# Wendison/FCL-taco2

Hardware: AMD Instinct MI355X
Metric: mel-frames/sec (FCL-taco2-S forward, batch=32, 80-mel) (higher is better)
Workload: dtype f32 via bf16x3-split MFMA operands, fp32 accumulate (max-abs 8e-6 on mel vs the reference; FCL_PRECISION=0 = exact fp32 MFMA)

## Files before the change

fcl-taco2_amd/csrc/decoder_step.hip:

```cpp
#include "fcl_common.h"
#include "lstm_epilogue.h"

namespace fcl {


template <int NT>
__device__ __forceinline__ void rowtile_mma(const float* A_l, int lda_l, const float* const (&wrow)[NT], int K, int r16, int kq,
                                            f32x4 (&out)[NT], int rot = 0) {
    f32x4 acc0[NT], acc1[NT];
#pragma unroll
    for (int t = 0; t < NT; ++t) acc0[t] = acc1[t] = (f32x4){0.f, 0.f, 0.f, 0.f};
    const float* ap = A_l + r16 * lda_l + kq * 4;
    const float* wp[NT];
#pragma unroll
    for (int t = 0; t < NT; ++t) wp[t] = wrow[t] + kq * 4;
    const int nfull = K >> 6;
    f32x4 bn[NT][4];
    int cc = nfull > 0 ? rot % nfull : 0;
    if (nfull > 0) {
#pragma unroll
        for (int t = 0; t < NT; ++t)
#pragma unroll
            for (int i = 0; i < 4; ++i) bn[t][i] = *reinterpret_cast<const f32x4*>(wp[t] + (cc << 6) + i * 16);
    }
// ... 253 lines not shown
            for (int e = 0; e < 4; ++e) split1(v[j][e], h[e], l[e]);
            *reinterpret_cast<uint2*>(Ah + r * ldk + c) = make_uint2(h[0] | ((unsigned)h[1] << 16), h[2] | ((unsigned)h[3] << 16));
            *reinterpret_cast<uint2*>(Al + r * ldk + c) = make_uint2(l[0] | ((unsigned)l[1] << 16), l[2] | ((unsigned)l[3] << 16));
        }
    }
    __device__ __forceinline__ void store(float* dst, int ld_l) const {
#pragma unroll
        for (int j = 0; j < 4; ++j) {
            const int i = threadIdx.x + j * 256, r = i >> 6, c = (i & 63) * 4;
            *reinterpret_cast<f32x4*>(dst + r * ld_l + c) = v[j];
        }
    }
};

__global__ __launch_bounds__(512) void feat_prenet_x3_kernel(const FeatPrenetArgs a) {
    const int M_feat = a.M_feat, M_pre = a.M_pre;
    const int Ms_feat = (a.live && a.t_prev >= 0) ? min(a.M_feat, a.live[a.t_prev]) : a.M_feat, Ms_pre = a.live ? min(a.M_pre, a.live[a.t_cur]) : a.M_pre;
    if (a.live && a.w0 && blockIdx.x == 0 && threadIdx.x == 0 && a.live[a.t_cur] > a.M_pre) atomicOr(a.status, (unsigned int)FCL_STATUS_ROWS_CAP);
    if ((int)blockIdx.x * (16) >= (a.h1 ? Ms_feat : Ms_pre)) return;
    extern __shared__ __attribute__((aligned(16))) float smem[];
    const int ldU = a.U + 8, ldO = a.O + 8, ldP = a.P + 8;
    u16* A1h = reinterpret_cast<u16*>(smem);
    u16* A1l = A1h + 16 * ldU;
    u16* A2h = A1l + 16 * ldU;
    u16* A2l = A2h + 16 * ldO;
    u16* A3h = A2l + 16 * ldO;
    u16* A3l = A3h + 16 * ldP;
    const int m0 = blockIdx.x * 16;
    const int lane = threadIdx.x & 63, wave = threadIdx.x >> 6, nwaves = blockDim.x >> 6;
    const int r16 = lane & 15, kq = lane >> 4;
    const int col = lane & 15, rq = lane >> 4;
    const unsigned int sbump = a.seed_dev ? *a.seed_dev * 0x9E3779B9u : 0u;
    const unsigned int seed0 = hash_u32(a.seed0 + sbump), seed1 = hash_u32(a.seed1 + sbump);

    const bool has_pre = a.w0 && m0 < M_pre;
    const int ptile = wave, ptile2 = wave + nwaves;
    const int nsU = (a.U + 31) >> 5, nsO = (a.O + 31) >> 5, nsP = (a.P + 31) >> 5, ptmax = ((a.P + 15) >> 4) - 1;
    const size_t lane8 = (size_t)lane * 8;
    auto frag = [&](const u16* base, int tile, int ns) { return base + (size_t)tile * ns * 512 + lane8; };
    float pb0[2] = {0.f, 0.f}, pb1[2] = {0.f, 0.f};
    if (has_pre) {
#pragma unroll
        for (int tt = 0; tt < 2; ++tt) {
            const int nc = min((tt ? ptile2 : ptile) * 16 + col, a.P - 1);
            pb0[tt] = a.b0[nc];
            pb1[tt] = a.b1[nc];
        }
    }
    if (a.h1) {
        f32x4 accv[1];
        load_rowtile_split(A1h, A1l, ldU, a.h1, a.U, a.U, m0, M_feat);
        __syncthreads();
        for (int tile = wave; tile * 16 < a.O; tile += nwaves) {
            const u16* const wh[1] = {frag(a.wf_hi, tile, nsU)};
            const u16* const wl[1] = {frag(a.wf_lo, tile, nsU)};
            const int nc = tile * 16 + col, ncc = min(nc, a.O - 1);
            float f0v[4];
            int fo[4];
#pragma unroll
            for (int r = 0; r < 4; ++r) {
                const int mc = min(m0 + rq * 4 + r, M_feat - 1);
                f0v[r] = a.F0[(size_t)mc * a.O + ncc];
                fo[r] = a.frame_off[mc];
            }
            rowtile_mma_x3<1>(A1h, A1l, ldU, wh, wl, a.U, r16, kq, accv);
#pragma unroll
            for (int r = 0; r < 4; ++r) {
                const int row = rq * 4 + r, m = m0 + row;
                float v = 0.f;
                if (m < Ms_feat && nc < a.O) {
                    v = accv[0][r] + f0v[r];
                    a.before[(size_t)(fo[r] + a.t_prev) * a.O + nc] = v;
                    if (a.before_p) store_p32(a.before_p, (a.O + 31) >> 5, fo[r] + a.t_prev, nc, v);
                }
                if (nc < a.O) split1((a.out_act && m < Ms_feat) ? act_apply(v, a.out_act) : v, A2h[row * ldO + nc], A2l[row * ldO + nc]);
            }
        }
        if (a.before_p && (a.O & 31)) {
            const int padc = 32 - (a.O & 31);
            for (int i = threadIdx.x; i < 16 * padc; i += blockDim.x) {
                const int m = m0 + i / padc;
                if (m < Ms_feat) store_p32(a.before_p, (a.O + 31) >> 5, a.frame_off[m] + a.t_prev, a.O + i % padc, 0.f);
            }
        }
    } else {
        for (int i = threadIdx.x; i < 16 * ldO; i += blockDim.x) { A2h[i] = 0; A2l[i] = 0; }
    }
    if (!has_pre) return;
    lds_barrier();
    if (a.teacher_in) {
        load_rowtile_split(A2h, A2l, ldO, a.teacher_in, a.teacher_ld, a.O, m0, M_pre);
        __syncthreads();
    }
    for (int tile = wave; tile * 16 < a.P; tile += 2 * nwaves) {
        const int tile2 = tile + nwaves;
        const u16* const wh[2] = {frag(a.w0_hi, tile, nsO), frag(a.w0_hi, min(tile2, ptmax), nsO)};
        const u16* const wl[2] = {frag(a.w0_lo, tile, nsO), frag(a.w0_lo, min(tile2, ptmax), nsO)};
        f32x4 accv[2];
        rowtile_mma_x3<2>(A2h, A2l, ldO, wh, wl, a.O, r16, kq, accv);
#pragma unroll
        for (int tt = 0; tt < 2; ++tt) {
            const int nc = (tt ? tile2 : tile) * 16 + col;
            if (nc < a.P) {
                const float bn = tile == ptile ? pb0[tt] : a.b0[nc];
#pragma unroll
                for (int r = 0; r < 4; ++r) {
                    const int row = rq * 4 + r, m = m0 + row;
                    float v = fmaxf(accv[tt][r] + bn, 0.f);
                    if (m < M_pre) v = drop_apply(v, a.drop_mode, a.keep0, a.P, m, nc, a.P, a.keep_scale, a.drop_p, seed0);
                    split1(v, A3h[row * ldP + nc], A3l[row * ldP + nc]);
                }
            }
        }
    }
    lds_barrier();
    for (int tile = wave; tile * 16 < a.P; tile += 2 * nwaves) {
        const int tile2 = tile + nwaves;
        const u16* const wh[2] = {frag(a.w1_hi, tile, nsP), frag(a.w1_hi, min(tile2, ptmax), nsP)};
        const u16* const wl[2] = {frag(a.w1_lo, tile, nsP), frag(a.w1_lo, min(tile2, ptmax), nsP)};
        f32x4 accv[2];
        rowtile_mma_x3<2>(A3h, A3l, ldP, wh, wl, a.P, r16, kq, accv);
#pragma unroll
        for (int tt = 0; tt < 2; ++tt) {
            const int nc = (tt ? tile2 : tile) * 16 + col;
            if (nc < a.P) {
                const float bn = tile == ptile ? pb1[tt] : a.b1[nc];
#pragma unroll
                for (int r = 0; r < 4; ++r) {
                    const int m = m0 + rq * 4 + r;
                    if (m >= Ms_pre) continue;
                    float v = fmaxf(accv[tt][r] + bn, 0.f);
                    v = drop_apply(v, a.drop_mode, a.keep1, a.P, m, nc, a.P, a.keep_scale, a.drop_p, seed1);
                    if (a.pre_out) a.pre_out[(size_t)m * a.P + nc] = v;
                    if (a.pre_out_p) store_p32(a.pre_out_p, (a.P + 31) >> 5, m, nc, v);
                    if (a.tap_prenet) a.tap_prenet[(size_t)(a.frame_off[m] + a.t_cur) * a.P + nc] = v;
                }
            }
        }
    }
}

__device__ __forceinline__ void p32_store4(unsigned short* __restrict__ p, int ld, long long m, int n, uint2 hi, uint2 lo) {
    unsigned short* line = p + ((size_t)m * ld + (n >> 5)) * 64 + (n & 31);
    *reinterpret_cast<uint2*>(line) = hi;
    *reinterpret_cast<uint2*>(line + 32) = lo;
}

struct OpsX3 {
    static constexpr bool kPlanes = true, kUnitsInLane = false;
    static constexpr int PAD = 16, LDS_BYTES = 2 * sizeof(u16);
    struct W {
        const u16 *hi, *lo;
        __device__ __forceinline__ W at(size_t o, size_t o2 = 0) const { return {hi + o + o2, lo + o + o2}; }
    };
    struct Tile {
        u16 *h, *l;
        __device__ __forceinline__ Tile at(int o) const { return {h + o, l + o}; }
        static __device__ __forceinline__ Tile carve(u16*& p, int n) {
            u16* b = p;
            p += 2 * n;
            return {b, b + n};
        }
        template <int N>
        static __device__ __forceinline__ Tile fixed() {
            __shared__ __attribute__((aligned(16))) u16 A_h[N];
            __shared__ __attribute__((aligned(16))) u16 A_lo[N];
            return {A_h, A_lo};
        }
    };
    template <int NT, int NS>
    struct Frag {
        s16x8 hi[NT][NS], lo[NT][NS];
        template <int S0 = 0, int S1 = NS>
        __device__ __forceinline__ void load(const W (&w)[NT]) {
#pragma unroll
            for (int t = 0; t < NT; ++t)
#pragma unroll
                for (int st = S0; st < S1; ++st) {
                    hi[t][st] = *reinterpret_cast<const s16x8*>(w[t].hi + st * 512);
                    lo[t][st] = *reinterpret_cast<const s16x8*>(w[t].lo + st * 512);
                }
        }
        template <bool W_IS_A>
        __device__ __forceinline__ void chain(Tile A, int ldk, int r16, int kq, f32x4 (&out)[NT]) const {
            auto mfma = [](s16x8 w, s16x8 a, f32x4 c) {
                return W_IS_A ? __builtin_amdgcn_mfma_f32_16x16x32_bf16(w, a, c, 0, 0, 0) : __builtin_amdgcn_mfma_f32_16x16x32_bf16(a, w, c, 0, 0, 0);
            };
            f32x4 acc[NT];
#pragma unroll
            for (int t = 0; t < NT; ++t) acc[t] = (f32x4){0.f, 0.f, 0.f, 0.f};
            const u16* ah = A.h + r16 * ldk + kq * 8;
            const u16* al = A.l + r16 * ldk + kq * 8;
#pragma unroll
            for (int st = 0; st < NS; ++st) {
                const s16x8 a_hi = *reinterpret_cast<const s16x8*>(ah + st * 32);
                const s16x8 a_lo = *reinterpret_cast<const s16x8*>(al + st * 32);
#pragma unroll
                for (int t = 0; t < NT; ++t) acc[t] = mfma(hi[t][st], a_lo, acc[t]);
#pragma unroll
                for (int t = 0; t < NT; ++t) acc[t] = mfma(lo[t][st], a_hi, acc[t]);
#pragma unroll
                for (int t = 0; t < NT; ++t) acc[t] = mfma(hi[t][st], a_hi, acc[t]);
            }
#pragma unroll
            for (int t = 0; t < NT; ++t) out[t] = acc[t];
        }
        __device__ __forceinline__ void mma_t(Tile A, int ldk, int r16, int kq, f32x4 (&out)[NT]) const { chain<true>(A, ldk, r16, kq, out); }
        __device__ __forceinline__ void mma_small(Tile A, int ldk, int r16, int kq, f32x4 (&out)[NT]) const { chain<false>(A, ldk, r16, kq, out); }
    };
    static __device__ __forceinline__ u16* dynamic_lds() {
        extern __shared__ __attribute__((aligned(16))) u16 x3_lds[];
        return x3_lds;
    }
    static __device__ __forceinline__ W wf(const FeatPrenetArgs& a) { return {a.wf_hi, a.wf_lo}; }
    static __device__ __forceinline__ W w0(const FeatPrenetArgs& a) { return {a.w0_hi, a.w0_lo}; }
    static __device__ __forceinline__ W w1(const FeatPrenetArgs& a) { return {a.w1_hi, a.w1_lo}; }
    static __device__ __forceinline__ W w(const GemmTerm& t) { return {t.Whi, t.Wlo}; }
    static __device__ __forceinline__ void store4(Tile t, int row, int ld, int col, const f32x4 v) {
        uint2 h, l;
        split4(v, h, l);
        *reinterpret_cast<uint2*>(t.h + row * ld + col) = h;
        *reinterpret_cast<uint2*>(t.l + row * ld + col) = l;
    }
    static __device__ __forceinline__ void store_rows(const RowTile256& r, Tile t, int ld) { r.split_store(t.h, t.l, ld); }
    static __device__ __forceinline__ void zero(Tile t, int n) {
        for (int i = threadIdx.x; i < n / 8; i += 512) {
            reinterpret_cast<uint4*>(t.h)[i] = make_uint4(0, 0, 0, 0);
            reinterpret_cast<uint4*>(t.l)[i] = make_uint4(0, 0, 0, 0);
        }
    }
};

struct OpsF32 {
    static constexpr bool kPlanes = false, kUnitsInLane = true;
    static constexpr int PAD = 8, LDS_BYTES = sizeof(float);
    struct W {
        const float* f;
        __device__ __forceinline__ W at(size_t o, size_t o2 = 0) const { return {f + o + o2}; }
    };
    struct Tile {
        float* p;
        __device__ __forceinline__ Tile at(int o) const { return {p + o}; }
        static __device__ __forceinline__ Tile carve(float*& p, int n) {
            float* b = p;
            p += n;
            return {b};
        }
        template <int N>
        static __device__ __forceinline__ Tile fixed() {
            __shared__ __attribute__((aligned(16))) float A_f[N];
            return {A_f};
        }
    };
    template <int NT, int NS>
    struct Frag {
        f32x4 w0[NT][NS], w1[NT][NS];
        template <int S0 = 0, int S1 = NS>
        __device__ __forceinline__ void load(const W (&w)[NT]) {
#pragma unroll
            for (int t = 0; t < NT; ++t)
#pragma unroll
                for (int st = S0; st < S1; ++st) {
                    w0[t][st] = *reinterpret_cast<const f32x4*>(w[t].f + st * 512);
                    w1[t][st] = *reinterpret_cast<const f32x4*>(w[t].f + st * 512 + 4);
                }
        }
        __device__ __forceinline__ void mma_t(Tile A, int ldk, int r16, int kq, f32x4 (&out)[NT]) const {
            f32x4 acc[NT];
#pragma unroll
            for (int t = 0; t < NT; ++t) acc[t] = (f32x4){0.f, 0.f, 0.f, 0.f};
            const float* a = A.p + r16 * ldk + kq * 4;
#pragma unroll
            for (int st = 0; st < NS; ++st) {
                const f32x4 a0 = *reinterpret_cast<const f32x4*>(a + st * 32), a1 = *reinterpret_cast<const f32x4*>(a + st * 32 + 16);
#pragma unroll
                for (int e = 0; e < 4; ++e)
#pragma unroll
                    for (int t = 0; t < NT; ++t) acc[t] = __builtin_amdgcn_mfma_f32_16x16x4f32(w0[t][st][e], a0[e], acc[t], 0, 0, 0);
#pragma unroll
                for (int e = 0; e < 4; ++e)
#pragma unroll
                    for (int t = 0; t < NT; ++t) acc[t] = __builtin_amdgcn_mfma_f32_16x16x4f32(w1[t][st][e], a1[e], acc[t], 0, 0, 0);
            }
#pragma unroll
            for (int t = 0; t < NT; ++t) out[t] = acc[t];
        }
        __device__ __forceinline__ void mma_small(Tile A, int ldk, int r16, int kq, f32x4 (&out)[NT]) const { mma_t(A, ldk, r16, kq, out); }
    };
    static __device__ __forceinline__ float* dynamic_lds() {
        extern __shared__ __attribute__((aligned(16))) float f32_lds[];
        return f32_lds;
    }
    static __device__ __forceinline__ W wf(const FeatPrenetArgs& a) { return {a.wf_ff}; }
    static __device__ __forceinline__ W w0(const FeatPrenetArgs& a) { return {a.w0_ff}; }
    static __device__ __forceinline__ W w1(const FeatPrenetArgs& a) { return {a.w1_ff}; }
    static __device__ __forceinline__ W w(const GemmTerm& t) { return {t.Wff}; }
    static __device__ __forceinline__ void store4(Tile t, int row, int ld, int col, const f32x4 v) { *reinterpret_cast<f32x4*>(t.p + row * ld + col) = v; }
    static __device__ __forceinline__ void store_rows(const RowTile256& r, Tile t, int ld) { r.store(t.p, ld); }
    static __device__ __forceinline__ void zero(Tile t, int n) {
        for (int i = threadIdx.x; i < n / 4; i += 512) reinterpret_cast<f32x4*>(t.p)[i] = (f32x4){0.f, 0.f, 0.f, 0.f};
    }
};

template <class Ops, int DROP, int RT>
__global__ __launch_bounds__(512) void feat_prenet_split_kernel(const FeatPrenetArgs a) {
    typedef typename Ops::Tile Tile;
    constexpr int SU = 8, SO = 3, SP = 8, U = 256, OP = 96, P = 256;
    const int M_feat = a.M_feat, M_pre = a.M_pre;
    int Ms_feat, Ms_pre;
    if (!feat_prenet_rows(a, 16 * RT, Ms_feat, Ms_pre)) return;
    constexpr int ldU = U + Ops::PAD, ldO = OP + Ops::PAD, ldP = P + Ops::PAD, ROWS = 16 * RT;
    static_assert(ldU == ldP, "the layer-1 operand tile re-uses the h1 tile's LDS");
    auto* lds = Ops::dynamic_lds();
    const Tile A1 = Tile::carve(lds, ROWS * ldU);
    const Tile A2 = Tile::carve(lds, ROWS * ldO);
    const Tile A3 = A1;
    const int O = a.O;
    const int m0 = blockIdx.x * ROWS;
    const int lane = threadIdx.x & 63, wave = __builtin_amdgcn_readfirstlane(threadIdx.x >> 6);
    const int r16 = lane & 15, kq = lane >> 4;
    const int arow = lane & 15, cq = lane >> 4;
    const bool has_feat = a.h1 != nullptr, has_pre = a.w0 != nullptr && m0 < M_pre;
    const bool feat_wave = has_feat && wave * 16 < O;
    const size_t lane8 = (size_t)lane * 8;
    auto frag = [&](const typename Ops::W w, int tile, int ns) { return w.at((size_t)tile * ns * 512, lane8); };
    const int t0 = wave, t1 = wave + 8;
    const int c1 = wave * 2;

    constexpr int HV = RT * 2;
    f32x4 hreg[HV];
    if (has_feat) {
#pragma unroll
        for (int j = 0; j < HV; ++j) {
            const int i = threadIdx.x + j * 512, r = i >> 6, c = (i & 63) * 4;
            hreg[j] = *reinterpret_cast<const f32x4*>(a.h1 + (size_t)min(m0 + r, M_feat - 1) * U + c);
        }
    }
    asm volatile("s_barrier" ::: "memory");
    typename Ops::template Frag<1, SU> ff;
    typename Ops::template Frag<2, SO> f0;
    typename Ops::template Frag<2, SP> f1;
    const int fnc = wave * 16 + cq * 4;
    f32x4 f0v[RT];
    int fo[RT];
    if (feat_wave) {
        const typename Ops::W w[1] = {frag(Ops::wf(a), wave, SU)};
        ff.load(w);
    }
#pragma unroll
    for (int q = 0; q < RT; ++q) {
        f0v[q] = (f32x4){0.f, 0.f, 0.f, 0.f};
        fo[q] = 0;
        if (feat_wave && fnc < O) {
            const int mc = min(m0 + q * 16 + arow, M_feat - 1);
            f0v[q] = *reinterpret_cast<const f32x4*>(a.F0 + (size_t)mc * O + fnc);
            fo[q] = a.frame_off[mc];
        }
    }
    unsigned int seed0 = 0, seed1 = 0;
    const unsigned int thr16 = (unsigned int)(a.drop_p * 65536.0f);
    if (DROP == 2) {
        const unsigned int sbump = a.seed_dev ? *a.seed_dev * 0x9E3779B9u : 0u;
        seed0 = hash_u32(a.seed0 + sbump);
        seed1 = hash_u32(a.seed1 + sbump);
    }
    f32x4 pb0[2], pb1[2];
    unsigned int k0[RT][2], k1[RT][2];
#pragma unroll
    for (int tt = 0; tt < 2; ++tt) pb0[tt] = (f32x4){0.f, 0.f, 0.f, 0.f};
    if (has_feat) asm volatile("s_barrier" ::: "memory");
    if (has_pre) {
        const typename Ops::W w[2] = {frag(Ops::w0(a), t0, SO), frag(Ops::w0(a), t1, SO)};
        f0.load(w);
#pragma unroll
        for (int tt = 0; tt < 2; ++tt) {
            const int nc = (tt ? t1 : t0) * 16 + cq * 4;
            pb0[tt] = *reinterpret_cast<const f32x4*>(a.b0 + nc);
            if (DROP == 1) {
#pragma unroll
                for (int q = 0; q < RT; ++q) k0[q][tt] = *reinterpret_cast<const unsigned int*>(a.keep0 + (size_t)min(m0 + q * 16 + arow, M_pre - 1) * P + nc);
            }
        }
    }
    Ops::zero(A2, ROWS * ldO);
    if (has_feat) {
#pragma unroll
        for (int j = 0; j < HV; ++j) {
            const int i = threadIdx.x + j * 512, r = i >> 6, c = (i & 63) * 4;
            Ops::store4(A1, r, ldU, c, hreg[j]);
        }
    }
#pragma unroll
    for (int tt = 0; tt < 2; ++tt) pb1[tt] = (f32x4){0.f, 0.f, 0.f, 0.f};
    auto request_l1 = [&]() {
        if (has_pre) {
            typename Ops::W w[2];
#pragma unroll
            for (int tt = 0; tt < 2; ++tt) w[tt] = frag(Ops::w1(a), c1 + tt, SP);
            f1.load(w);
#pragma unroll
            for (int tt = 0; tt < 2; ++tt) {
                const int nc = (c1 + tt) * 16 + cq * 4;
                pb1[tt] = *reinterpret_cast<const f32x4*>(a.b1 + nc);
                if (DROP == 1) {
#pragma unroll
                    for (int q = 0; q < RT; ++q) k1[q][tt] = *reinterpret_cast<const unsigned int*>(a.keep1 + (size_t)min(m0 + q * 16 + arow, M_pre - 1) * P + nc);
                }
            }
        }
    };
    lds_barrier();
    if (feat_wave) {
#pragma unroll
        for (int q = 0; q < RT; ++q) {
            f32x4 accv[1];
            ff.mma_t(A1.at(q * 16 * ldU), ldU, r16, kq, accv);
            const int row = q * 16 + arow, m = m0 + row;
            if (fnc < O) {
                f32x4 v = (f32x4){0.f, 0.f, 0.f, 0.f};
                if (m < Ms_feat) {
                    v = accv[0] + f0v[q];
                    const long long fr = (long long)fo[q] + a.t_prev;
                    *reinterpret_cast<f32x4*>(a.before + (size_t)fr * O + fnc) = v;
                    if constexpr (Ops::kPlanes) {
                        if (a.before_p) {
                            uint2 h, l;
                            split4(v, h, l);
                            p32_store4(a.before_p, (O + 31) >> 5, fr, fnc, h, l);
                        }
                    }
                    if (a.out_act) {
#pragma unroll
                        for (int r = 0; r < 4; ++r) v[r] = act_apply(v[r], a.out_act);
                    }
                }
                Ops::store4(A2, row, ldO, fnc, v);
            }
        }
    }
    if (Ops::kPlanes && has_feat && a.before_p && (O & 31)) {
        const int padc = 32 - (O & 31);
        for (int i = threadIdx.x; i < ROWS * padc; i += 512) {
            const int m = m0 + i / padc;
            if (m < Ms_feat) store_p32(a.before_p, (O + 31) >> 5, a.frame_off[m] + a.t_prev, O + i % padc, 0.f);
        }
    }
    if (!has_pre) return;
    request_l1();
    lds_barrier();
    if constexpr (Ops::kPlanes) {
        if (a.teacher_in) {
#pragma unroll
            for (int q = 0; q < RT; ++q) load_rowtile_split(A2.h + q * 16 * ldO, A2.l + q * 16 * ldO, ldO, a.teacher_in, a.teacher_ld, O, m0 + q * 16, M_pre);
            lds_barrier();
        }
    }
#pragma unroll
    for (int q = 0; q < RT; ++q) {
        f32x4 accv[2];
        f0.mma_t(A2.at(q * 16 * ldO), ldO, r16, kq, accv);
        const int row = q * 16 + arow, m = m0 + row;
#pragma unroll
        for (int tt = 0; tt < 2; ++tt) {
            const int nc = (tt ? t1 : t0) * 16 + cq * 4;
            f32x4 v = accv[tt] + pb0[tt];
#pragma unroll
            for (int r = 0; r < 4; ++r) v[r] = fmaxf(v[r], 0.f);
            v = drop4<DROP>(v, DROP == 1 ? k0[q][tt] : 0u, (unsigned int)m * (unsigned int)P + (unsigned int)nc, seed0, thr16, a.keep_scale);
            Ops::store4(A3, row, ldP, nc, v);
        }
    }
    lds_barrier();
#pragma unroll
    for (int q = 0; q < RT; ++q) {
        f32x4 accv[2];
        f1.mma_t(A3.at(q * 16 * ldP), ldP, r16, kq, accv);
        const int m = m0 + q * 16 + arow;
        if (m >= Ms_pre) continue;
#pragma unroll
        for (int tt = 0; tt < 2; ++tt) {
            const int nc = (c1 + tt) * 16 + cq * 4;
            f32x4 v = accv[tt] + pb1[tt];
#pragma unroll
            for (int r = 0; r < 4; ++r) v[r] = fmaxf(v[r], 0.f);
            v = drop4<DROP>(v, DROP == 1 ? k1[q][tt] : 0u, (unsigned int)m * (unsigned int)P + (unsigned int)nc, seed1, thr16, a.keep_scale);
            if (a.pre_out) *reinterpret_cast<f32x4*>(a.pre_out + (size_t)m * P + nc) = v;
            if constexpr (Ops::kPlanes) {
                if (a.pre_out_p) {
                    uint2 h, l;
                    split4(v, h, l);
                    p32_store4(a.pre_out_p, SP, m, nc, h, l);
                }
            }
            if (a.tap_prenet) *reinterpret_cast<f32x4*>(a.tap_prenet + (size_t)(a.frame_off[m] + a.t_cur) * P + nc) = v;
        }
    }
}


__device__ __forceinline__ void gates_to_cell(const LstmStepArgs& a, int g, int lane, const f32x4& acc, bool units_in_lane, int m, int u, bool valid, int Ms,
                                              const CellIn& ci) {
    __shared__ float g_l[4][16][17];
    const int lo = lane & 15, hi = lane >> 4;
#pragma unroll
    for (int i = 0; i < 4; ++i) {
        if (units_in_lane) g_l[g][lo][hi * 4 + i] = acc[i];
        else g_l[g][hi * 4 + i][lo] = acc[i];
    }
    __syncthreads();
    if (!valid || m >= Ms) return;
    const int row = threadIdx.x >> 4, uc = threadIdx.x & 15;
    const float pre[4] = {g_l[0][row][uc], g_l[1][row][uc], g_l[2][row][uc], g_l[3][row][uc]};
    cell_finish(a, m, u, pre, ci);
}

constexpr int kSmallStepsAtEntry = 4;

template <class Ops, int NT>
__device__ __forceinline__ f32x4 small_walk(const LstmStepArgs& a, typename Ops::Tile A, int ldk, int m0, int M, int g, int u0, int lane) {
    const int r16 = lane & 15, kq = lane >> 4;
    RowTile256 rows[NT];
#pragma unroll
    for (int t = 0; t < NT; ++t) rows[t].request(a.term[t].A, a.term[t].lda, m0, M);
    asm volatile("s_barrier" ::: "memory");
    const size_t fo = (size_t)((g * a.U + u0) >> 4) * 8 * 512 + (size_t)lane * 8;
    typename Ops::template Frag<1, 8> wf[NT];
    const typename Ops::W w0[1] = {Ops::w(a.term[0]).at(fo)}, w1[1] = {Ops::w(a.term[NT - 1]).at(fo)};
    wf[0].load(w0);
    if (NT > 1) wf[NT - 1].template load<0, kSmallStepsAtEntry>(w1);
    __builtin_amdgcn_sched_barrier(0);
#pragma unroll
    for (int t = 0; t < NT; ++t) Ops::store_rows(rows[t], A.at(t * 256), ldk);
    asm volatile("" ::: "memory");
    if (NT > 1) wf[NT - 1].template load<kSmallStepsAtEntry, 8>(w1);
    __syncthreads();
    f32x4 acc = {0.f, 0.f, 0.f, 0.f};
#pragma unroll
    for (int t = 0; t < NT; ++t) {
        f32x4 part[1];
        wf[t].mma_small(A.at(t * 256), ldk, r16, kq, part);
        acc += part[0];
    }
    return acc;
}

template <class Ops>
__global__ __launch_bounds__(256) void lstm_small_resident_kernel(const LstmStepArgs a) {
    const int M = a.M, Ms = live_rows_of(a.M, a.m_dev);
    if ((int)blockIdx.y * 16 >= Ms) return;
    constexpr int LD = 512 + Ops::PAD;
    const typename Ops::Tile A = Ops::Tile::template fixed<16 * LD>();
    const int m0 = blockIdx.y * 16, u0 = blockIdx.x * 16;
    const int lane = threadIdx.x & 63, g = threadIdx.x >> 6;
    const int erow = threadIdx.x >> 4, euc = threadIdx.x & 15;
    const int em = m0 + erow, eu = u0 + euc;
    const bool evalid = em < M && eu < a.U;
    CellIn ci;
    if (evalid) ci = cell_prefetch(a, em, eu);
    const f32x4 acc = a.nterms == 2 ? small_walk<Ops, 2>(a, A, LD, m0, M, g, u0, lane) : small_walk<Ops, 1>(a, A, LD, m0, M, g, u0, lane);
    gates_to_cell(a, g, lane, acc, Ops::kUnitsInLane, em, eu, evalid, Ms, ci);
}

__global__ __launch_bounds__(256) void lstm_small_x3_kernel(const LstmStepArgs a) {
    const int M = a.M, Ms = live_rows_of(a.M, a.m_dev);
    if ((int)blockIdx.y * 16 >= Ms) return;
    constexpr int KC = 512;
    __shared__ __attribute__((aligned(16))) u16 A_h[16 * (KC + 16)];
    __shared__ __attribute__((aligned(16))) u16 A_lo[16 * (KC + 16)];
    const int m0 = blockIdx.y * 16, u0 = blockIdx.x * 16;
    const int lane = threadIdx.x & 63, g = threadIdx.x >> 6;
    const int r16 = lane & 15, kq = lane >> 4;
    const int erow = threadIdx.x >> 4, euc = threadIdx.x & 15;
    const int em = m0 + erow, eu = u0 + euc;
    const bool evalid = em < M && eu < a.U;
    CellIn ci;
    if (evalid) ci = cell_prefetch(a, em, eu);
    f32x4 acc = {0.f, 0.f, 0.f, 0.f};
    for (int t = 0; t < a.nterms; ++t) {
        const GemmTerm T = a.term[t];
        for (int k0 = 0; k0 < T.K; k0 += KC) {
            const int kc = min(KC, T.K - k0);
            __syncthreads();
            load_rowtile_split(A_h, A_lo, kc + 16, T.A + k0, T.lda, kc, m0, M);
            __syncthreads();
            const size_t fo = ((size_t)((g * a.U + u0) >> 4) * ((T.K + 31) >> 5) + (k0 >> 5)) * 512 + (size_t)lane * 8;
            const u16* const wh[1] = {T.Whi + fo};
            const u16* const wl[1] = {T.Wlo + fo};
            f32x4 part[1];
            rowtile_mma_x3<1>(A_h, A_lo, kc + 16, wh, wl, kc, r16, kq, part);
            acc += part[0];
        }
    }
    gates_to_cell(a, g, lane, acc, false, em, eu, evalid, Ms, ci);
}


constexpr int SMALL_KC = 512;

__device__ __forceinline__ void lstm_small_body(const LstmStepArgs& a) {
    const int M = a.M, Ms = live_rows_of(a.M, a.m_dev);
    if ((int)blockIdx.y * 16 >= Ms) return;
    __shared__ __attribute__((aligned(16))) float A_l[16 * (SMALL_KC + 4)];
    __shared__ float g_l[4][16][17];
    const int m0 = blockIdx.y * 16, u0 = blockIdx.x * 16;
    const int lane = threadIdx.x & 63, g = threadIdx.x >> 6;
    const int r16 = lane & 15, kq = lane >> 4;
    const int u = u0 + r16;
    f32x4 acc = {0.f, 0.f, 0.f, 0.f};
    for (int t = 0; t < a.nterms; ++t) {
        const GemmTerm T = a.term[t];
        for (int k0 = 0; k0 < T.K; k0 += SMALL_KC) {
            const int kc = min(SMALL_KC, T.K - k0);
            __syncthreads();
            load_rowtile(A_l, kc + 4, T.A + k0, T.lda, kc, m0, M);
            __syncthreads();
            const float* const wr[1] = {T.W + (size_t)(g * a.U + min(u, a.U - 1)) * T.ldw + k0};
            f32x4 part[1];
            rowtile_mma<1>(A_l, kc + 4, wr, kc, r16, kq, part, blockIdx.y);
            acc += part[0];
        }
    }
    {
        const int col = lane & 15, rq = lane >> 4;
#pragma unroll
        for (int r = 0; r < 4; ++r) g_l[g][rq * 4 + r][col] = acc[r];
    }
    __syncthreads();
    const int row = threadIdx.x >> 4, uc = threadIdx.x & 15;
    const int m = m0 + row, uu = u0 + uc;
    if (m >= Ms || uu >= a.U) return;
    const CellIn ci = cell_prefetch(a, m, uu);
    const float pre[4] = {g_l[0][row][uc], g_l[1][row][uc], g_l[2][row][uc], g_l[3][row][uc]};
    cell_finish(a, m, uu, pre, ci);
}

__global__ __launch_bounds__(256) void lstm_small_kernel(const LstmStepArgs a) { lstm_small_body(a); }

__global__ __launch_bounds__(256) void lstm_small_pair_kernel(const LstmStepArgs a0, const LstmStepArgs a1) {
    if (blockIdx.z == 0) lstm_small_body(a0);
    else lstm_small_body(a1);
}

int launch_lstm_small(const LstmStepArgs& a, hipStream_t s) {
    const double fl = lstm_step_flops(a);
    dim3 grid((a.U + 15) / 16, (a.M + 15) / 16);
    bool planes = true;
    for (int i = 0; i < a.nterms; ++i) planes = planes && a.term[i].Whi && a.term[i].Wlo && (a.term[i].K & 7) == 0 && a.term[i].ldw == a.term[i].K;
    planes = planes && (a.U & 15) == 0;
    bool pre256 = a.nterms == 2 || (a.nterms == 1 && !a.h_in), ff = true;
    for (int i = 0; i < a.nterms; ++i) {
        pre256 = pre256 && a.term[i].K == 256;
        ff = ff && a.term[i].Wff != nullptr;
    }
    if (planes) {
        ProfScope ps("lstm_small_kernel/bf16x3", fl, a.M, s);
        if (pre256) hipLaunchKernelGGL(lstm_small_resident_kernel<OpsX3>, grid, dim3(256), 0, s, a);
        else hipLaunchKernelGGL(lstm_small_x3_kernel, grid, dim3(256), 0, s, a);
    } else if (pre256 && ff && (a.U & 15) == 0) {
        ProfScope ps("lstm_small_ff_kernel/f32", fl, a.M, s);
        hipLaunchKernelGGL(lstm_small_resident_kernel<OpsF32>, grid, dim3(256), 0, s, a);
    } else {
        ProfScope ps("lstm_small_kernel", fl, a.M, s);
        hipLaunchKernelGGL(lstm_small_kernel, grid, dim3(256), 0, s, a);
    }
    return check_hip(hipGetLastError(), "lstm_small launch");
}

int launch_lstm_small_pair(const LstmStepArgs& a0, const LstmStepArgs& a1, hipStream_t s) {
    const double fl = lstm_step_flops(a0) + lstm_step_flops(a1);
    const int mmax = a0.M > a1.M ? a0.M : a1.M;
    dim3 grid((a0.U + 15) / 16, (mmax + 15) / 16, 2);
    ProfScope ps("lstm_small_pair_kernel", fl, a0.M + a1.M, s);
    hipLaunchKernelGGL(lstm_small_pair_kernel, grid, dim3(256), 0, s, a0, a1);
    return check_hip(hipGetLastError(), "lstm_small_pair launch");
}

int launch_lstm_small_pair_any(const LstmStepArgs& a0, const LstmStepArgs& a1, hipStream_t s, bool* handled) {
    *handled = false;
    if (a0.U != a1.U || a0.m_dev || a1.m_dev) return 0;
    for (const LstmStepArgs* a : {&a0, &a1})
        for (int i = 0; i < a->nterms; ++i)
            if (!a->term[i].A || !a->term[i].W || a->term[i].Whi || a->term[i].Wff) return 0;
    *handled = true;
    return launch_lstm_small_pair(a0, a1, s);
}

static int launch_fp_drop(const void* const (&fn)[3], int drop_mode, dim3 grid, size_t lds, const FeatPrenetArgs& a, hipStream_t s) {
    const void* f = fn[drop_mode == 1 || drop_mode == 2 ? drop_mode : 0];
    const int rc = ensure_dyn_lds(f, (int)lds);
    if (rc) return rc;
    void* args[] = {const_cast<FeatPrenetArgs*>(&a)};
    return check_hip(hipLaunchKernel(f, grid, dim3(512), args, lds, s), "feat_prenet launch");
}

template <class Ops, int RT>
static int launch_feat_prenet_split(const FeatPrenetArgs& a, int rows, hipStream_t s) {
    constexpr size_t lds_s = (size_t)Ops::LDS_BYTES * 16 * RT * ((256 + Ops::PAD) + (96 + Ops::PAD));
    static const void* const fn[3] = {reinterpret_cast<const void*>(feat_prenet_split_kernel<Ops, 0, RT>), reinterpret_cast<const void*>(feat_prenet_split_kernel<Ops, 1, RT>),
                                      reinterpret_cast<const void*>(feat_prenet_split_kernel<Ops, 2, RT>)};
    return launch_fp_drop(fn, a.drop_mode, dim3((rows + 16 * RT - 1) / (16 * RT), 1), lds_s, a, s);
}

int launch_feat_prenet(const FeatPrenetArgs& a, hipStream_t s) {
    const int rows = a.h1 ? a.M_feat : a.M_pre;
    if (rows <= 0) return 0;
    FCL_REQUIRE(!(a.U & 3) && !(a.O & 3) && !(a.P & 3), FCL_ERR_SHAPE, "feat_prenet: U/O/P must be multiples of 4");
    const size_t lds = sizeof(float) * 16 * ((size_t)(a.U + 4) + (a.O + 4) + (a.P + 4));
    FCL_REQUIRE(lds <= 160 * 1024, FCL_ERR_SHAPE, "feat_prenet: tile does not fit LDS (%zu B)", lds);
    double fl = 0;
    if (a.h1) fl += 2.0 * a.M_feat * a.O * a.U;
    if (a.w0) fl += 2.0 * a.M_pre * ((double)a.P * a.O + (double)a.P * a.P);
    const bool planes = a.wf_hi && a.wf_lo && a.w0_hi && a.w0_lo && a.w1_hi && a.w1_lo && !(a.U & 7) && !(a.O & 7) && !(a.P & 7);
    FCL_REQUIRE(planes || (!a.pre_out_p && !a.before_p), FCL_ERR_INVALID, "feat_prenet: P32 outputs need the bf16x3 weight planes");
    FCL_REQUIRE(!a.w0 || a.pre_out || a.pre_out_p, FCL_ERR_INVALID, "feat_prenet: no prenet output buffer");
    FCL_REQUIRE(!a.pre_out_p || !(a.P & 31), FCL_ERR_SHAPE, "feat_prenet: P32 prenet output needs P %% 32 == 0");
    if (planes) {
        ProfScope ps("feat_prenet_kernel/bf16x3", fl, rows, s);
        if (a.U == 256 && a.O > 64 && a.O <= 96 && a.P == 256) {
            const int rc = rows >= 4096 ? launch_feat_prenet_split<OpsX3, 2>(a, rows, s) : launch_feat_prenet_split<OpsX3, 1>(a, rows, s);
            if (rc) return rc;
        } else {
            const size_t lds3 = 2 * sizeof(unsigned short) * 16 * ((size_t)(a.U + 8) + (a.O + 8) + (a.P + 8));
            const int rc = ensure_dyn_lds(reinterpret_cast<const void*>(feat_prenet_x3_kernel), 160 * 1024);
            if (rc) return rc;
            hipLaunchKernelGGL(feat_prenet_x3_kernel, dim3((rows + 15) / 16), dim3(512), lds3, s, a);
        }
    } else if (a.wf_ff && a.w0_ff && a.w1_ff && a.U == 256 && a.P == 256 && a.O > 64 && a.O <= 96 && !a.teacher_in && !a.pre_out_p && !a.before_p &&
               (!a.w0 || a.pre_out)) {
        ProfScope ps("feat_prenet_split_kernel/f32", fl, rows, s);
        const int rc = launch_feat_prenet_split<OpsF32, 1>(a, rows, s);
        if (rc) return rc;
    } else {
        ProfScope ps("feat_prenet_kernel", fl, rows, s);
        const int rc = ensure_dyn_lds(reinterpret_cast<const void*>(feat_prenet_kernel), 160 * 1024);
        if (rc) return rc;
        hipLaunchKernelGGL(feat_prenet_kernel, dim3((rows + 15) / 16), dim3(512), lds, s, a);
    }
    return check_hip(hipGetLastError(), "feat_prenet launch");
}

}
```

Measured before the change: 54.47 million.

## Add multi-tile walk kernel for feat/prenet with LDS-resident weights and double buffering

Adds a feat_prenet_walk kernel in which each workgroup handles several 16-row tiles. The feature-projection weights are loaded once into LDS with global_load_lds, and the row tiles are double-buffered so the next tile's loads overlap the current tile's MFMA work. The prenet biases are staged in LDS and the P32 padding stores are folded into the main loop. It is selected for mid-size row counts (at least 112 tiles and fewer than 4096 rows) through FP_WALK_TILES and FP_WALK_MIN_TILES. It also adds compile-time-gated s_memtime instrumentation for profiling each phase; in exchange the kernel uses more LDS and has fewer workgroups to spread across the chip.

Result: faster. 55.54 million (median of 6 runs) (+2.0%).

```diff
diff --git a/fcl-taco2_amd/csrc/decoder_step.hip b/fcl-taco2_amd/csrc/decoder_step.hip
--- a/fcl-taco2_amd/csrc/decoder_step.hip
+++ b/fcl-taco2_amd/csrc/decoder_step.hip
@@ -579,6 +579,34 @@
     }
 };
 
+#ifdef FCL_FP_TS
+constexpr int kFpTsWorkgroups = 1024;
+__device__ long long g_fp_ts[kFpTsWorkgroups * 8 * 8];
+struct FpStamps {
+    long long t[8] = {0, 0, 0, 0, 0, 0, 0, 0};
+    template <int I>
+    __device__ __forceinline__ void at(bool drain = false) {
+        __builtin_amdgcn_sched_barrier(0);
+        if (drain) asm volatile("s_waitcnt vmcnt(0)" ::: "memory");
+        asm volatile("s_memtime %0\n\ts_waitcnt lgkmcnt(0)" : "=s"(t[I])::"memory");
+        __builtin_amdgcn_sched_barrier(0);
+    }
+    __device__ __forceinline__ void flush() {
+        at<7>();
+        if ((threadIdx.x & 63) == 0 && blockIdx.x < kFpTsWorkgroups) {
+#pragma unroll
+            for (int i = 0; i < 8; ++i) g_fp_ts[(blockIdx.x * 8 + (threadIdx.x >> 6)) * 8 + i] = t[i];
+        }
+    }
+};
+#define FP_STAMP(ts, i, ...) ts.at<i>(__VA_ARGS__)
+#define FP_STAMP_FLUSH(ts) ts.flush()
+#else
+struct FpStamps {};
+#define FP_STAMP(ts, i, ...)
+#define FP_STAMP_FLUSH(ts)
+#endif
+
 template <class Ops, int DROP, int RT>
 __global__ __launch_bounds__(512) void feat_prenet_split_kernel(const FeatPrenetArgs a) {
     typedef typename Ops::Tile Tile;
@@ -586,6 +614,8 @@
     const int M_feat = a.M_feat, M_pre = a.M_pre;
     int Ms_feat, Ms_pre;
     if (!feat_prenet_rows(a, 16 * RT, Ms_feat, Ms_pre)) return;
+    [[maybe_unused]] FpStamps ts;
+    FP_STAMP(ts, 0);
     constexpr int ldU = U + Ops::PAD, ldO = OP + Ops::PAD, ldP = P + Ops::PAD, ROWS = 16 * RT;
     static_assert(ldU == ldP, "the layer-1 operand tile re-uses the h1 tile's LDS");
     auto* lds = Ops::dynamic_lds();
@@ -667,6 +697,7 @@
             Ops::store4(A1, r, ldU, c, hreg[j]);
         }
     }
+    FP_STAMP(ts, 1);
 #pragma unroll
     for (int tt = 0; tt < 2; ++tt) pb1[tt] = (f32x4){0.f, 0.f, 0.f, 0.f};
     auto request_l1 = [&]() {
@@ -687,6 +718,7 @@
         }
     };
     lds_barrier();
+    FP_STAMP(ts, 2);
     if (feat_wave) {
 #pragma unroll
         for (int q = 0; q < RT; ++q) {
@@ -722,7 +754,11 @@
             if (m < Ms_feat) store_p32(a.before_p, (O + 31) >> 5, a.frame_off[m] + a.t_prev, O + i % padc, 0.f);
         }
     }
-    if (!has_pre) return;
+    FP_STAMP(ts, 3);
+    if (!has_pre) {
+        FP_STAMP_FLUSH(ts);
+        return;
+    }
     request_l1();
     lds_barrier();
     if constexpr (Ops::kPlanes) {
@@ -732,6 +768,7 @@
             lds_barrier();
         }
     }
+    FP_STAMP(ts, 4);
 #pragma unroll
     for (int q = 0; q < RT; ++q) {
         f32x4 accv[2];
@@ -748,6 +785,8 @@
         }
     }
     lds_barrier();
+    FP_STAMP(ts, 5);
+    FP_STAMP(ts, 6, true);
 #pragma unroll
     for (int q = 0; q < RT; ++q) {
         f32x4 accv[2];
@@ -772,8 +811,237 @@
             if (a.tap_prenet) *reinterpret_cast<f32x4*>(a.tap_prenet + (size_t)(a.frame_off[m] + a.t_cur) * P + nc) = v;
         }
     }
-}
-
+    FP_STAMP_FLUSH(ts);
+}
+
+__device__ __forceinline__ void glds16_unseen(const void* g, const void* l) {
+    typedef const __attribute__((address_space(3))) void* lds_t;
+    const unsigned dst = __builtin_amdgcn_readfirstlane((unsigned)(uintptr_t)(lds_t)l);
+    unsigned keep;
+    asm volatile("s_mov_b32 %0, m0\n\ts_mov_b32 m0, %2\n\ts_nop 0\n\tglobal_load_lds_dwordx4 %1, off\n\ts_mov_b32 m0, %0" : "=&s"(keep) : "v"(g), "s"(dst) : "memory");
+}
+
+template <int DROP, bool FEAT, bool PRE>
+__device__ __forceinline__ void feat_prenet_walk(const FeatPrenetArgs& a, const int ntw, const int Ms_feat, const int Ms_pre) {
+    typedef OpsX3 Ops;
+    typedef Ops::Tile Tile;
+    constexpr int SU = 8, SO = 3, SP = 8, U = 256, OP = 96, P = 256;
+    constexpr int ldU = U + Ops::PAD, ldO = OP + Ops::PAD, ldP = P + Ops::PAD;
+    constexpr int BUF = 2 * 16 * (ldU + ldO);
+    static_assert(ldU == ldP, "the layer-1 operand tile re-uses the h1 tile's LDS");
+    const int M_feat = a.M_feat, M_pre = a.M_pre;
+    [[maybe_unused]] FpStamps ts;
+    FP_STAMP(ts, 0);
+    const int O = a.O;
+    const int lane = threadIdx.x & 63, wave = __builtin_amdgcn_readfirstlane(threadIdx.x >> 6);
+    const int r16 = lane & 15, kq = lane >> 4;
+    const int arow = lane & 15, cq = lane >> 4;
+    constexpr bool has_feat = FEAT, pre_any = PRE;
+    const bool feat_wave = has_feat && wave * 16 < O;
+    const int mbeg = blockIdx.x * 16 * ntw;
+    const int nt = min(ntw, ((has_feat ? Ms_feat : Ms_pre) - mbeg + 15) >> 4);
+    u16* lds = Ops::dynamic_lds();
+    u16* const WF = lds + wave * (2 * SU * 512);
+    lds += ((O + 15) >> 4) * (2 * SU * 512);
+    const Tile A1 = Tile::carve(lds, 16 * ldU);
+    const Tile A2 = Tile::carve(lds, 16 * ldO);
+    float* const BL = reinterpret_cast<float*>(lds + BUF);
+    const size_t lane8 = (size_t)lane * 8;
+    auto frag = [&](const Ops::W w, int tile, int ns) { return w.at((size_t)tile * ns * 512, lane8); };
+    const int t0 = wave, t1 = wave + 8;
+    const int c1 = wave * 2;
+    const int fnc = wave * 16 + cq * 4;
+    const int padc = O + wave * 16 + cq * 4;
+    const bool pad_lane = wave < 2 && padc < ((O + 31) & ~31);
+
+    f32x4 hrow[2];
+    f32x4 f0v = (f32x4){0.f, 0.f, 0.f, 0.f};
+    int fo = 0;
+    unsigned int k0[2] = {0u, 0u}, k1[2] = {0u, 0u};
+    auto request_rows = [&](int m0) {
+        if (has_feat) {
+#pragma unroll
+            for (int j = 0; j < 2; ++j) {
+                const int i = threadIdx.x + j * 512, r = i >> 6, c = (i & 63) * 4;
+                hrow[j] = *reinterpret_cast<const f32x4*>(a.h1 + (unsigned)(min(m0 + r, M_feat - 1) * U + c));
+            }
+        }
+    };
+    auto request_feat = [&](int m0) {
+        if (feat_wave && fnc < O) {
+            const int mc = min(m0 + arow, M_feat - 1);
+            f0v = *reinterpret_cast<const f32x4*>(a.F0 + (unsigned)(mc * O + fnc));
+            fo = a.frame_off[(unsigned)mc];
+        }
+    };
+    auto request_keep = [&](unsigned int (&k)[2], const uint8_t* keep, int m0, int ca, int cb) {
+        if (DROP == 1 && pre_any && m0 < M_pre) {
+            const unsigned mk = (unsigned)(min(m0 + arow, M_pre - 1) * P);
+            k[0] = *reinterpret_cast<const unsigned int*>(keep + mk + ca * 16 + cq * 4);
+            k[1] = *reinterpret_cast<const unsigned int*>(keep + mk + cb * 16 + cq * 4);
+        }
+    };
+    auto store_rows = [&](int buf) {
+        Ops::zero(A2.at(buf * BUF), 16 * ldO);
+        if (has_feat) {
+#pragma unroll
+            for (int j = 0; j < 2; ++j) {
+                const int i = threadIdx.x + j * 512, r = i >> 6, c = (i & 63) * 4;
+                Ops::store4(A1.at(buf * BUF), r, ldU, c, hrow[j]);
+            }
+        }
+    };
+
+    if (feat_wave) {
+        const Ops::W w = frag(Ops::wf(a), wave, SU);
+#pragma unroll
+        for (int st = 0; st < SU; ++st) {
+            glds16_unseen(w.hi + st * 512, WF + st * 512);
+            glds16_unseen(w.lo + st * 512, WF + (SU + st) * 512);
+        }
+    }
+    request_rows(mbeg);
+    asm volatile("s_barrier" ::: "memory");
+    request_feat(mbeg);
+    request_keep(k0, a.keep0, mbeg, t0, t1);
+    request_keep(k1, a.keep1, mbeg, c1, c1 + 1);
+    Ops::Frag<2, SO> f0;
+    Ops::Frag<2, SP> f1;
+    unsigned int seed0 = 0, seed1 = 0;
+    const unsigned int thr16 = (unsigned int)(a.drop_p * 65536.0f);
+    if (DROP == 2) {
+        const unsigned int sbump = a.seed_dev ? *a.seed_dev * 0x9E3779B9u : 0u;
+        seed0 = hash_u32(a.seed0 + sbump);
+        seed1 = hash_u32(a.seed1 + sbump);
+    }
+    f32x4 bias = (f32x4){0.f, 0.f, 0.f, 0.f};
+    const bool bias_thread = pre_any && threadIdx.x < 2 * (P / 4);
+    if (pre_any) {
+        if (bias_thread) bias = *reinterpret_cast<const f32x4*>((threadIdx.x < P / 4 ? a.b0 : a.b1 - P) + threadIdx.x * 4);
+        const Ops::W w0[2] = {frag(Ops::w0(a), t0, SO), frag(Ops::w0(a), t1, SO)};
+        f0.load(w0);
+        const Ops::W w1[2] = {frag(Ops::w1(a), c1, SP), frag(Ops::w1(a), c1 + 1, SP)};
+        f1.load(w1);
+    }
+    store_rows(0);
+    if (bias_thread) *reinterpret_cast<f32x4*>(BL + threadIdx.x * 4) = bias;
+    FP_STAMP(ts, 1);
+
+    auto tile = [&](const int q) {
+        const int buf = q & 1, m0 = mbeg + q * 16;
+        const Tile T1 = A1.at(buf * BUF), T2 = A2.at(buf * BUF);
+        const bool has_pre = pre_any && m0 < M_pre;
+        lds_barrier();
+        if (q == 0) FP_STAMP(ts, 2);
+        if (feat_wave) {
+            f32x4 acc = (f32x4){0.f, 0.f, 0.f, 0.f};
+            const u16* ah = T1.h + r16 * ldU + kq * 8;
+            const u16* al = T1.l + r16 * ldU + kq * 8;
+            const u16* wf = WF + lane8;
+#pragma unroll
+            for (int st = 0; st < SU; ++st) {
+                const s16x8 a_hi = *reinterpret_cast<const s16x8*>(ah + st * 32), a_lo = *reinterpret_cast<const s16x8*>(al + st * 32);
+                const s16x8 w_hi = *reinterpret_cast<const s16x8*>(wf + st * 512), w_lo = *reinterpret_cast<const s16x8*>(wf + (SU + st) * 512);
+                acc = __builtin_amdgcn_mfma_f32_16x16x32_bf16(w_hi, a_lo, acc, 0, 0, 0);
+                acc = __builtin_amdgcn_mfma_f32_16x16x32_bf16(w_lo, a_hi, acc, 0, 0, 0);
+                acc = __builtin_amdgcn_mfma_f32_16x16x32_bf16(w_hi, a_hi, acc, 0, 0, 0);
+            }
+            const int m = m0 + arow;
+            if (fnc < O) {
+                f32x4 v = (f32x4){0.f, 0.f, 0.f, 0.f};
+                if (m < Ms_feat) {
+                    v = acc + f0v;
+                    const long long fr = (long long)fo + a.t_prev;
+                    *reinterpret_cast<f32x4*>(a.before + (size_t)fr * O + fnc) = v;
+                    if (a.before_p) {
+                        uint2 h, l;
+                        split4(v, h, l);
+                        p32_store4(a.before_p, (O + 31) >> 5, fr, fnc, h, l);
+                        if (pad_lane) p32_store4(a.before_p, (O + 31) >> 5, fr, padc, make_uint2(0u, 0u), make_uint2(0u, 0u));
+                    }
+                    if (a.out_act) {
+#pragma unroll
+                        for (int r = 0; r < 4; ++r) v[r] = act_apply(v[r], a.out_act);
+                    }
+                }
+                Ops::store4(T2, arow, ldO, fnc, v);
+            }
+        }
+        request_rows(m0 + 16);
+        request_feat(m0 + 16);
+        if (q == 0) FP_STAMP(ts, 3);
+        f32x4 out1[2];
+        if (has_pre) {
+            lds_barrier();
+            if (a.teacher_in) {
+                load_rowtile_split(T2.h, T2.l, ldO, a.teacher_in, a.teacher_ld, O, m0, M_pre);
+                lds_barrier();
+            }
+            if (q == 0) FP_STAMP(ts, 4);
+            {
+                f32x4 accv[2];
+                f0.mma_t(T2, ldO, r16, kq, accv);
+                const int m = m0 + arow;
+#pragma unroll
+                for (int tt = 0; tt < 2; ++tt) {
+                    const int nc = (tt ? t1 : t0) * 16 + cq * 4;
+                    f32x4 v = accv[tt] + *reinterpret_cast<const f32x4*>(BL + nc);
+#pragma unroll
+                    for (int r = 0; r < 4; ++r) v[r] = fmaxf(v[r], 0.f);
+                    v = drop4<DROP>(v, DROP == 1 ? k0[tt] : 0u, (unsigned int)m * (unsigned int)P + (unsigned int)nc, seed0, thr16, a.keep_scale);
+                    Ops::store4(T1, arow, ldP, nc, v);
+                }
+            }
+            request_keep(k0, a.keep0, m0 + 16, t0, t1);
+            lds_barrier();
+            if (q == 0) {
+                FP_STAMP(ts, 5);
+                FP_STAMP(ts, 6, true);
+            }
+            f1.mma_t(T1, ldP, r16, kq, out1);
+        }
+        store_rows(buf ^ 1);
+        asm volatile("" : "+v"(f0v), "+v"(fo), "+v"(k0[0]), "+v"(k0[1]));
+        if (has_pre) {
+            const int m = m0 + arow;
+            if (m < Ms_pre) {
+#pragma unroll
+                for (int tt = 0; tt < 2; ++tt) {
+                    const int nc = (c1 + tt) * 16 + cq * 4;
+                    f32x4 v = out1[tt] + *reinterpret_cast<const f32x4*>(BL + P + nc);
+#pragma unroll
+                    for (int r = 0; r < 4; ++r) v[r] = fmaxf(v[r], 0.f);
+                    v = drop4<DROP>(v, DROP == 1 ? k1[tt] : 0u, (unsigned int)m * (unsigned int)P + (unsigned int)nc, seed1, thr16, a.keep_scale);
+                    if (a.pre_out) *reinterpret_cast<f32x4*>(a.pre_out + (size_t)m * P + nc) = v;
+                    if (a.pre_out_p) {
+                        uint2 h, l;
+                        split4(v, h, l);
+                        p32_store4(a.pre_out_p, SP, m, nc, h, l);
+                    }
+                    if (a.tap_prenet) *reinterpret_cast<f32x4*>(a.tap_prenet + (size_t)(a.frame_off[m] + a.t_cur) * P + nc) = v;
+                }
+            }
+            request_keep(k1, a.keep1, m0 + 16, c1, c1 + 1);
+        }
+    };
+    tile(0);
+#pragma unroll 1
+    for (int q = 1; q < nt; ++q) tile(q);
+    FP_STAMP_FLUSH(ts);
+}
+
+template <int DROP>
+__global__ __launch_bounds__(512) void feat_prenet_walk_kernel(const FeatPrenetArgs a, const int ntw) {
+    int Ms_feat, Ms_pre;
+    if (!feat_prenet_rows(a, 16 * ntw, Ms_feat, Ms_pre)) return;
+    const bool pre = a.w0 != nullptr && (int)blockIdx.x * 16 * ntw < a.M_pre;
+    if (a.h1 != nullptr) {
+        if (pre) feat_prenet_walk<DROP, true, true>(a, ntw, Ms_feat, Ms_pre);
+        else feat_prenet_walk<DROP, true, false>(a, ntw, Ms_feat, Ms_pre);
+    } else if (pre) {
+        feat_prenet_walk<DROP, false, true>(a, ntw, Ms_feat, Ms_pre);
+    }
+}
 
 __device__ __forceinline__ void gates_to_cell(const LstmStepArgs& a, int g, int lane, const f32x4& acc, bool units_in_lane, int m, int u, bool valid, int Ms,
                                               const CellIn& ci) {
@@ -962,12 +1230,53 @@
     return launch_lstm_small_pair(a0, a1, s);
 }
 
-static int launch_fp_drop(const void* const (&fn)[3], int drop_mode, dim3 grid, size_t lds, const FeatPrenetArgs& a, hipStream_t s) {
+static int launch_fp_drop(const void* const (&fn)[3], int drop_mode, dim3 grid, size_t lds, const FeatPrenetArgs& a, hipStream_t s, int ntw = 0) {
     const void* f = fn[drop_mode == 1 || drop_mode == 2 ? drop_mode : 0];
     const int rc = ensure_dyn_lds(f, (int)lds);
     if (rc) return rc;
-    void* args[] = {const_cast<FeatPrenetArgs*>(&a)};
-    return check_hip(hipLaunchKernel(f, grid, dim3(512), args, lds, s), "feat_prenet launch");
+    void* args1[] = {const_cast<FeatPrenetArgs*>(&a)};
+    void* args2[] = {const_cast<FeatPrenetArgs*>(&a), &ntw};
+    return check_hip(hipLaunchKernel(f, grid, dim3(512), ntw ? args2 : args1, lds, s), "feat_prenet launch");
+}
+
+#ifdef FCL_FP_TS
+static void print_fp_stamps(const char* form, int rows, int wgs) {
+    static const int want = tunable("FP_TS", 0);
+    if (!want) return;
+    if (hipDeviceSynchronize() != hipSuccess) return;
+    static long long h[kFpTsWorkgroups * 64];
+    if (hipMemcpyFromSymbol(h, HIP_SYMBOL(g_fp_ts), sizeof(h)) != hipSuccess) return;
+    double sum[8] = {}, mx[8] = {};
+    int cnt[8] = {};
+    for (int w = 0; w < (wgs < kFpTsWorkgroups ? wgs : kFpTsWorkgroups) * 8; ++w) {
+        const long long* t = &h[(size_t)w * 8];
+        if (!t[0]) continue;
+        for (int i = 1; i < 8; ++i) {
+            if (!t[i] || (i == 3 && (w & 7) >= 5)) continue;
+            const double d = (double)(t[i] - t[0]);
+            sum[i] += d; cnt[i]++;
+            if (d > mx[i]) mx[i] = d;
+        }
+    }
+    fprintf(stderr, "fp_ts %s rows %d workgroups %d: cycles since entry, mean (max):", form, rows, wgs);
+    static const char* const name[8] = {"", "rows->LDS", "barrier0", "phase1", "barrier1", "phase2+barrier2", "all landed", "exit"};
+    for (int i = 1; i < 8; ++i) fprintf(stderr, "  %s %.0f (%.0f)", name[i], cnt[i] ? sum[i] / cnt[i] : 0.0, mx[i]);
+    fprintf(stderr, "\n");
+    void* p = nullptr;
+    if (hipGetSymbolAddress(&p, HIP_SYMBOL(g_fp_ts)) == hipSuccess) (void)hipMemset(p, 0, sizeof(h));
+}
+#else
+static void print_fp_stamps(const char*, int, int) {}
+#endif
+
+static int launch_feat_prenet_walk(const FeatPrenetArgs& a, int rows, int ntw, hipStream_t s) {
+    const size_t lds_w = sizeof(u16) * ((size_t)((a.O + 15) / 16) * 2 * 8 * 512 + 2 * 2 * 16 * ((256 + OpsX3::PAD) + (96 + OpsX3::PAD))) + 2 * 256 * sizeof(float);
+    static const void* const fn[3] = {reinterpret_cast<const void*>(feat_prenet_walk_kernel<0>), reinterpret_cast<const void*>(feat_prenet_walk_kernel<1>),
+                                      reinterpret_cast<const void*>(feat_prenet_walk_kernel<2>)};
+    const int tiles = (rows + 15) / 16, wgs = (tiles + ntw - 1) / ntw;
+    const int rc = launch_fp_drop(fn, a.drop_mode, dim3(wgs, 1), lds_w, a, s, ntw);
+    if (!rc) print_fp_stamps("walk", rows, wgs);
+    return rc;
 }
 
 template <class Ops, int RT>
@@ -975,7 +1284,10 @@
     constexpr size_t lds_s = (size_t)Ops::LDS_BYTES * 16 * RT * ((256 + Ops::PAD) + (96 + Ops::PAD));
     static const void* const fn[3] = {reinterpret_cast<const void*>(feat_prenet_split_kernel<Ops, 0, RT>), reinterpret_cast<const void*>(feat_prenet_split_kernel<Ops, 1, RT>),
                                       reinterpret_cast<const void*>(feat_prenet_split_kernel<Ops, 2, RT>)};
-    return launch_fp_drop(fn, a.drop_mode, dim3((rows + 16 * RT - 1) / (16 * RT), 1), lds_s, a, s);
+    const int wgs = (rows + 16 * RT - 1) / (16 * RT);
+    const int rc = launch_fp_drop(fn, a.drop_mode, dim3(wgs, 1), lds_s, a, s);
+    if (!rc && Ops::kPlanes) print_fp_stamps(RT == 2 ? "split RT=2" : "split RT=1", rows, wgs);
+    return rc;
 }
 
 int launch_feat_prenet(const FeatPrenetArgs& a, hipStream_t s) {
@@ -992,8 +1304,14 @@
     FCL_REQUIRE(!a.w0 || a.pre_out || a.pre_out_p, FCL_ERR_INVALID, "feat_prenet: no prenet output buffer");
     FCL_REQUIRE(!a.pre_out_p || !(a.P & 31), FCL_ERR_SHAPE, "feat_prenet: P32 prenet output needs P %% 32 == 0");
     if (planes) {
-        ProfScope ps("feat_prenet_kernel/bf16x3", fl, rows, s);
-        if (a.U == 256 && a.O > 64 && a.O <= 96 && a.P == 256) {
+        const bool resident = a.U == 256 && a.O > 64 && a.O <= 96 && a.P == 256;
+        static const int walk_tiles = tunable("FP_WALK_TILES", 2), walk_min = tunable("FP_WALK_MIN_TILES", 112);
+        const bool walk = resident && walk_tiles > 0 && rows < 4096 && (rows + 15) / 16 >= walk_min;
+        ProfScope ps(walk ? "feat_prenet_walk_kernel/bf16x3" : "feat_prenet_kernel/bf16x3", fl, rows, s);
+        if (walk) {
+            const int rc = launch_feat_prenet_walk(a, rows, walk_tiles, s);
+            if (rc) return rc;
+        } else if (resident) {
             const int rc = rows >= 4096 ? launch_feat_prenet_split<OpsX3, 2>(a, rows, s) : launch_feat_prenet_split<OpsX3, 1>(a, rows, s);
             if (rc) return rc;
         } else {
```
